# renjie-liang/HUAL

Measured on AMD Instinct MI355X. Metric: train clips/sec, higher is better.
Workload: dtype f32 (fp16x3 / bf16x3 split-operand MFMA, fp32 accumulate); 1 GPU; Charades-STA SeqPAN train step (fwd+bwd+clip+AdamWD, dropout 0.2), batch 64/GPU, T=128, vdim=1024, L=20, C=8, dim=128, 8 heads, 2 attention layers, random init; ONE batch resident in HBM, batch assembly (hual_assemble_batch) outside the timed region; global_batch=64, T=128, vdim=1024, L=20, parallelism=dp1, launch=hipGraph, video_dtype=f32

## Files before the change

### hual_amd/csrc/dablock.h

```cpp
#pragma once
#include "common.h"
#include "rowops.h"

namespace hual {

#define HUAL_LNPROJ_MAX 5
struct LnProjArgs {
  const float* x;
  const float* xa; int pre_site; float* x_out;
  uint8_t* pre_bits; uint8_t* y1_bits;
  const float* x2;
  const float* g1; const float* b1; float* y1;
  int drop_site1;
  const float* g2; const float* b2; float* y2;
  float* mean; float* rstd;
  int nproj;
  const float* wimg[HUAL_LNPROJ_MAX];
  const float* bias[HUAL_LNPROJ_MAX];
  float* out[HUAL_LNPROJ_MAX]; int ldo[HUAL_LNPROJ_MAX];
  int src[HUAL_LNPROJ_MAX];
  int accum[HUAL_LNPROJ_MAX];
  int act[HUAL_LNPROJ_MAX];
  int out_site[HUAL_LNPROJ_MAX];
  uint8_t* out_bits[HUAL_LNPROJ_MAX];
// ... 35 lines not shown
  int nsteps;
  const float* A[HUAL_LNBWD_MAX]; int lda[HUAL_LNBWD_MAX];
  const uint8_t* a_bits[HUAL_LNBWD_MAX];
  float* a_save[HUAL_LNBWD_MAX];
  const float* wimg_t[HUAL_LNBWD_MAX];
  int dst[HUAL_LNBWD_MAX];
  const float* add_dy1;
  const uint8_t* dy1_bits;
  const float* x; const float* mean; const float* rstd;
  const float* g1; const float* g2;
  const float* add1;
  float* dx;
  float* dz; const uint8_t* dz_bits;
  float* part;
  int R; int MT; uint32_t drop_row0;
  int Nv;
  const float* pre_x; const float* pre_mean; const float* pre_rstd; const float* pre_g; const float* pre_dy; const float* pre_add;
};
int ln_proj_bwd_rows(int R, int Nv = 0);
int ln_proj_bwd_blocks(int R, int Nv = 0);
int launch_ln_proj_bwd(const LnProjBwdArgs& a, const DropCfg& drop, hipStream_t s);

struct DaMidBwdArgs {
  const float* dz1;
  const float *gate, *val, *sg, *xg, *sv, *xv;
  const float* w[10];
  float *d_sc, *d_val, *d_ln1a, *d_g, *dz_sg, *dz_xg, *d_sv, *d_xv, *d_satt, *d_xatt;
  int R; int MT; int Nv;
};
int launch_da_mid_bwd(const DaMidBwdArgs& a, hipStream_t s);
bool ln2_mid_bwd_fits(const LnProjBwdArgs& a, const DaMidBwdArgs& m);
int launch_ln2_mid_bwd(const LnProjBwdArgs& a, const DaMidBwdArgs& m, const DropCfg& drop, hipStream_t s);

}
```

### hual_amd/csrc/dablock.hip

```cpp
#include "dablock.h"
#include "tilecore.h"
#include "prof.h"

using namespace hual;

__device__ __forceinline__ float4 sig4(float4 v) { return make_float4(sigmoidf_(v.x), sigmoidf_(v.y), sigmoidf_(v.z), sigmoidf_(v.w)); }

#include "lnproj_body.h"

template <int NT, bool PLAIN>
__global__ __launch_bounds__(CB_THREADS) void ln_proj_kernel(LnProjArgs a, DropCfg drop) {
  extern __shared__ __attribute__((aligned(16))) char lp_lds[];
  ln_proj_body<NT, false, PLAIN>(a, drop, lp_lds);
}
template <int NT>
__global__ __launch_bounds__(CB_THREADS) void ln_proj_pair_kernel(LnProjArgs a0, LnProjArgs a1, DropCfg drop) {
  extern __shared__ __attribute__((aligned(16))) char lp_lds[];
  if (blockIdx.y == 0) ln_proj_body<NT>(a0, drop, lp_lds);
  else ln_proj_body<NT>(a1, drop, lp_lds);
}

#define DA_ST_NT st4
#define DP_ROWS 48
#define DP_PLANE (DP_ROWS * 256)
// ... 248 lines not shown
    uint32_t nbe[NT];
#pragma unroll
    for (int rt = 0; rt < NT; ++rt) nbe[rt] = 15u;
    if (dr.enabled) drop_rows((uint32_t)(a.site + 4), a.bits4, nbe);
#pragma unroll
    for (int rt = 0; rt < NT; ++rt) {
      float4 v = addb(T1[rt], 8);
      if (dr.enabled) v = drop_scale(nbe[rt], v, dr.scale);
      v = cb_add(v, SV[rt]);
      save(a.out, rt, v);
      if (TAIL) scratch[(16 * rt + j) * 32 + (ecol >> 2)] = v;
    }
  }
  if (TAIL) {
    lds_barrier();
    ln_proj_body<NT, true, true>(*lp, drop, P1, r0, scratch, r0, 32, DP_ROWS, TP);
  }
}
template <int NT>
__global__ __launch_bounds__(CB_THREADS) void da_post_kernel(DaPostArgs a, DropCfg drop) {
  extern __shared__ __attribute__((aligned(16))) char dp_lds[];
  da_post_body<NT, false>(a, drop, nullptr, dp_lds);
}
template <int NT>
__global__ __launch_bounds__(CB_THREADS) void da_post_lnproj_kernel(DaPostArgs a, DropCfg drop, LnProjArgs lp) {
  extern __shared__ __attribute__((aligned(16))) char dp_lds[];
  da_post_body<NT, true>(a, drop, &lp, dp_lds);
}

#define LB_ROWS 48
#define LB_U (LB_ROWS / 16)
template <int NT> struct DaMidPre { TfW wa, wb; float4 gate[NT], val[NT]; };
#define LB_LDS ((size_t)4 * LB_ROWS * 256 + 8 * 4 * 32 * 16 + 2 * LB_ROWS * sizeof(float))
template <bool PRE, int NT, bool SIX, bool MID>
__device__ __forceinline__ bool ln_proj_bwd_body(const LnProjBwdArgs& a, const DropCfg& drop, char* lb_lds, const DaMidBwdArgs* m,
                                                 DaMidPre<NT>* mp, float4 (&zv)[LB_U]) {
  char* S0 = lb_lds;
  char* S1 = S0 + 2 * LB_ROWS * 256;
  char* Ps = S1 + 2 * LB_ROWS * 256;
  float* ainv0 = reinterpret_cast<float*>(Ps + 8 * 4 * 32 * 16);
  float* ainv1 = ainv0 + LB_ROWS;
  const int lane = threadIdx.x & 63, wave = threadIdx.x >> 6;
  const int l32 = threadIdx.x & 31, grp = threadIdx.x >> 5;
  const int col = 4 * l32;
  const int MT = a.MT, R = a.R;
  const int tile_ = xcd_tile_clip(blockIdx.x, R, a.Nv, MT);
  if (tile_ < 0) return false;
  const int r0 = tile_ * MT;
  const int RE = min(R, r0 + MT);
  const int j = lane & 15, g = lane >> 4, ecol = 16 * wave + 4 * g;
  const DropRegs dr = drop_load(drop);

  TfW w[2];
  tf_load_w(w[0], a.wimg_t[0], wave, lane);
  float4 nv[LB_U], xv[LB_U], a1v[LB_U];
  float mu[LB_U], rsd[LB_U];
  constexpr bool pre = PRE;
  const float* add1p = pre ? (a.pre_add ? a.pre_add : a.x) : (a.add1 ? a.add1 : a.x);
  const float* a0p = pre ? a.pre_dy : a.A[0];
  const int lda0 = pre ? HUAL_D : a.lda[0];
  uint32_t nkb[LB_U];
  const int nsteps = SIX ? 6 : (MID ? 1 : a.nsteps);
  auto has_bits = [&](int k) { return !SIX && a.a_bits[k] != nullptr; };
  auto to_second = [&](int k) { return SIX ? k >= 4 : a.dst[k] != 0; };
  const bool has_g2 = SIX || (!MID && a.g2 != nullptr), has_add_dy1 = SIX || (!MID && a.add_dy1 != nullptr), has_dy1_bits = !SIX && a.dy1_bits != nullptr;
  const uint8_t* kb0p = has_bits(0) ? a.a_bits[0] : reinterpret_cast<const uint8_t*>(a.x);
  float4 pxv[LB_U];
  float pmu[LB_U], prs[LB_U];
#pragma unroll
  for (int u = 0; u < LB_U; ++u) {
    const int row = min(r0 + grp + 16 * u, R - 1);
    nv[u] = ld4(a0p + (size_t)row * lda0 + col);
    nkb[u] = SIX ? 0u : kb0p[(size_t)row * 16 + (l32 >> 1)];
    xv[u] = ld4(a.x + (size_t)row * HUAL_D + col);
    a1v[u] = ld4(add1p + (size_t)row * HUAL_D + col);
    mu[u] = a.mean[row];
    rsd[u] = a.rstd[row];
    if (pre) { pxv[u] = ld4(a.pre_x + (size_t)row * HUAL_D + col); pmu[u] = a.pre_mean[row]; prs[u] = a.pre_rstd[row]; }
  }
  const float4 g1 = ld4(a.g1 + col);
  float4 sg2 = f4zero(), sb2 = f4zero();
  if (pre) {
    const float4 pg = ld4(a.pre_g + col);
#pragma unroll
    for (int u = 0; u < LB_U; ++u) {
      const int lr = grp + 16 * u;
      const bool ok = lr < MT && r0 + lr < RE;
      const float4 v = pxv[u], dy = nv[u];
      const float mean = pmu[u], rstd = prs[u];
      const float4 xh = make_float4((v.x - mean) * rstd, (v.y - mean) * rstd, (v.z - mean) * rstd, (v.w - mean) * rstd);
      if (ok) { sb2 = cb_add(sb2, dy); sg2 = cb_fma(dy, xh, sg2); }
      const float4 gv = cb_mul(dy, pg);
      const float m1 = fast_sum32(cb_hsum(gv)) * (1.0f / HUAL_D);
      const float m2 = fast_sum32(cb_hsum(cb_mul(gv, xh))) * (1.0f / HUAL_D);
      float4 dx = make_float4(rstd * (gv.x - m1 - xh.x * m2), rstd * (gv.y - m1 - xh.y * m2),
                              rstd * (gv.z - m1 - xh.z * m2), rstd * (gv.w - m1 - xh.w * m2));
      if (a.pre_add) dx = make_float4(__fadd_rn(dx.x, a1v[u].x), __fadd_rn(dx.y, a1v[u].y), __fadd_rn(dx.z, a1v[u].z), __fadd_rn(dx.w, a1v[u].w));
      nv[u] = dx;
      a1v[u] = dx;
    }
  }
  const float4 g2 = has_g2 ? ld4(a.g2 + col) : f4zero();
  float4 addt[NT];
  const float* addp = has_add_dy1 ? a.add_dy1 : a.x;
#pragma unroll
  for (int rt = 0; rt < NT; ++rt) addt[rt] = (SIX || MID) ? f4zero() : ld4(addp + (uint32_t)min(r0 + 16 * rt + j, R - 1) * (uint32_t)HUAL_D + (uint32_t)ecol);
  auto fill = [&](int k) {
    char* S = (k & 1) ? S1 : S0;
    float* ai = (k & 1) ? ainv1 : ainv0;
#pragma unroll
    for (int u = 0; u < LB_U; ++u) {
      const int lr = grp + 16 * u, row = r0 + lr;
      if (lr >= MT) continue;
      const bool ok = row < RE;
      float4 v = ok ? nv[u] : f4zero();
      if (has_bits(k)) {
// ... 326 lines not shown
  tf_mma_lean<NT, DP_PLANE>(P2, wb, lane, accp);
  tf_load_w(wb, a.w[9], wave, lane);
  fold(T2, ainv2, true);
#pragma unroll
  for (int rt = 0; rt < NT; ++rt) {
    T1[rt] = cb_add(T1[rt], U3[rt]);
    T2[rt] = cb_add(T2[rt], U4[rt]);
    save_nt(a.d_sv, rt, T1[rt]);
    save_nt(a.d_xv, rt, T2[rt]);
  }
  zero_invalid(T1);
  zero_invalid(T2);
  put_max(smaxA, T1);
  put_max(smaxB, T2);
  lds_barrier();
  put_planes(P1, ainv1, smaxA, T1);
  put_planes(P0, ainv0, smaxB, T2);
  lds_barrier();
  tf_mma_lean<NT, DP_PLANE>(P1, wa, lane, accp);
  fold(T1, ainv1, true);
#pragma unroll
  for (int rt = 0; rt < NT; ++rt) save(a.d_satt, rt, T1[rt]);
  tf_mma_lean<NT, DP_PLANE>(P0, wb, lane, accp);
  fold(T2, ainv0, true);
#pragma unroll
  for (int rt = 0; rt < NT; ++rt) save(a.d_xatt, rt, T2[rt]);
}
template <int NT>
__global__ __launch_bounds__(CB_THREADS) void da_mid_bwd_kernel(DaMidBwdArgs a) {
  extern __shared__ __attribute__((aligned(16))) char dm_lds[];
  const float4 zin[3] = {};
  da_mid_bwd_body<NT, false>(a, dm_lds, nullptr, zin);
}
template <int NT>
__global__ __launch_bounds__(CB_THREADS) void ln2_mid_bwd_kernel(LnProjBwdArgs a, DaMidBwdArgs m, DropCfg drop) {
  extern __shared__ __attribute__((aligned(16))) char lm_lds[];
  DaMidPre<NT> mp;
  float4 zv[LB_U];
  if (!ln_proj_bwd_body<false, NT, false, true>(a, drop, lm_lds, &m, &mp, zv)) return;
  static_assert(DP_SLOT == 2 * LB_ROWS * 256, "the middle's slot 1 must be the first body's slot 1");
  da_mid_bwd_body<NT, true>(m, lm_lds, &mp, zv);
}

#if defined(HUAL_STAMPS) && (HUAL_STAMPS == 1 || (HUAL_STAMPS >= 4 && HUAL_STAMPS <= 6))
extern "C" int hual_debug_stamps(unsigned long long* out, int n) {
  return (int)hipMemcpyFromSymbol(out, HIP_SYMBOL(g_hual_stamps), sizeof(unsigned long long) * (size_t)n);
}
extern "C" int hual_debug_stamps_reset() {
  static unsigned long long zeros[512 * HUAL_STAMP_SLOTS];
  return (int)hipMemcpyToSymbol(HIP_SYMBOL(g_hual_stamps), zeros, sizeof(zeros));
}
#endif

namespace hual {

static int tile_rows(int R, int Nv, int max_rows) { return xcd_clip_rows(R, Nv, 16, max_rows); }
int ln_proj_rows(int R, int Nv) { return tile_rows(R, Nv, LP_ROWS); }
int ln_proj_pair_rows(int R) {
  int mt = 16;
  while (mt < LP_ROWS && 2 * xcd_clip_grid(R, 0, mt) > 256) ++mt;
  return mt;
}
int da_post_rows(int R, int Nv) { return tile_rows(R, Nv, DP_ROWS); }

static int check_ln_proj(const LnProjArgs& a) {
  HUAL_REQUIRE(a.x && a.g1 && a.b1 && a.y1 && a.mean && a.rstd && a.R > 0, "ln_proj: null / empty");
// ... 156 lines not shown
  HUAL_CHECK_HIP(hipGetLastError());
  return 0;
}

static int check_da_mid_bwd(const DaMidBwdArgs& a) {
  HUAL_REQUIRE(a.dz1 && a.gate && a.val && a.sg && a.xg && a.sv && a.xv && a.R > 0, "da_mid_bwd: null / empty");
  HUAL_REQUIRE(a.MT >= 1 && a.MT <= DP_ROWS, "da_mid_bwd: MT must be 1..48");
  for (int k = 0; k < 10; ++k) HUAL_REQUIRE(a.w[k] != nullptr, "da_mid_bwd: null weight image");
  HUAL_REQUIRE(a.d_sc && a.d_val && a.d_ln1a && a.d_g && a.dz_sg && a.dz_xg && a.d_sv && a.d_xv && a.d_satt && a.d_xatt, "da_mid_bwd: null output");
  return 0;
}
static void da_mid_bwd_work(const DaMidBwdArgs& a, double& flops, double& bytes) {
  const double rows = (double)a.R;
  flops += 10.0 * 2.0 * rows * HUAL_D * HUAL_D;
  bytes += 4.0 * (rows * HUAL_D * 17.0 + 10.0 * HUAL_D * HUAL_D);
}

int launch_da_mid_bwd(const DaMidBwdArgs& a, hipStream_t s) {
  int rc = check_da_mid_bwd(a);
  if (rc) return rc;
  const size_t lds = DM_LDS;
  double flops = 0.0, bytes = 0.0;
  da_mid_bwd_work(a, flops, bytes);
  const dim3 grid(xcd_clip_grid(a.R, a.Nv, a.MT));
  switch (cdiv(a.MT, 16)) {
    case 1: { HUAL_DYN_LDS(da_mid_bwd_kernel<1>, 160 * 1024); HUAL_LAUNCH(flops, bytes, da_mid_bwd_kernel<1>, grid, dim3(CB_THREADS), lds, s, a); break; }
    case 2: { HUAL_DYN_LDS(da_mid_bwd_kernel<2>, 160 * 1024); HUAL_LAUNCH(flops, bytes, da_mid_bwd_kernel<2>, grid, dim3(CB_THREADS), lds, s, a); break; }
    default: { HUAL_DYN_LDS(da_mid_bwd_kernel<3>, 160 * 1024); HUAL_LAUNCH(flops, bytes, da_mid_bwd_kernel<3>, grid, dim3(CB_THREADS), lds, s, a); break; }
  }
  HUAL_CHECK_HIP(hipGetLastError());
  return 0;
}

bool ln2_mid_bwd_fits(const LnProjBwdArgs& a, const DaMidBwdArgs& m) {
  return a.nsteps == 1 && !a.pre_x && !a.g2 && !a.add_dy1 && a.dst[0] == 0 && a.dz && a.dz == m.dz1 && a.R == m.R && a.Nv == m.Nv && a.MT == m.MT;
}

int launch_ln2_mid_bwd(const LnProjBwdArgs& a, const DaMidBwdArgs& m, const DropCfg& drop, hipStream_t s) {
  int rc = check_ln_proj_bwd(a);
  if (rc) return rc;
  if ((rc = check_da_mid_bwd(m))) return rc;
  HUAL_REQUIRE(ln2_mid_bwd_fits(a, m), "ln2_mid_bwd: one product into one layer norm whose dz is the middle's dz1, on the same row tiles");
  static_assert(LB_ROWS == DP_ROWS, "the two bodies share their row tiles");
  const size_t lds = LB_LDS > DM_LDS ? LB_LDS : DM_LDS;
  double flops = 0.0, bytes = 0.0;
  ln_proj_bwd_work(a, flops, bytes);
  da_mid_bwd_work(m, flops, bytes);
  bytes -= 4.0 * (double)a.R * HUAL_D;
  const dim3 grid(xcd_clip_grid(a.R, a.Nv, a.MT));
  switch (cdiv(a.MT, 16)) {
    case 1: { HUAL_DYN_LDS(ln2_mid_bwd_kernel<1>, 160 * 1024); HUAL_LAUNCH(flops, bytes, ln2_mid_bwd_kernel<1>, grid, dim3(CB_THREADS), lds, s, a, m, drop); break; }
    case 2: { HUAL_DYN_LDS(ln2_mid_bwd_kernel<2>, 160 * 1024); HUAL_LAUNCH(flops, bytes, ln2_mid_bwd_kernel<2>, grid, dim3(CB_THREADS), lds, s, a, m, drop); break; }
    default: { HUAL_DYN_LDS(ln2_mid_bwd_kernel<3>, 160 * 1024); HUAL_LAUNCH(flops, bytes, ln2_mid_bwd_kernel<3>, grid, dim3(CB_THREADS), lds, s, a, m, drop); break; }
  }
  HUAL_CHECK_HIP(hipGetLastError());
  return 0;
}

}
```

### hual_amd/csrc/prof.cpp

```cpp
#include <stdlib.h>
#include "prof.h"
#include <map>
#include <string>
#include <vector>
#include <string.h>
#include "../../include/hual_seqpan.h"

namespace hual {

namespace {
struct Rec { std::string name; hipEvent_t a, b; double flops, bytes; };
struct Agg { std::string name; int64_t launches = 0; double usec = 0.0, flops = 0.0, bytes = 0.0; };
struct State {
  bool on = false;
  std::vector<Rec> recs;
  std::vector<Agg> aggs;
};
thread_local State g_prof;

std::string clean(const char* s) {
  std::string n(s);
  while (!n.empty() && (n.front() == '(' || n.front() == ' ')) n.erase(n.begin());
  while (!n.empty() && (n.back() == ')' || n.back() == ' ')) n.pop_back();
  return n;
// ... 39 lines not shown
    auto it = idx.find(r.name);
    if (it == idx.end()) {
      it = idx.emplace(r.name, g_prof.aggs.size()).first;
      g_prof.aggs.push_back(Agg{r.name});
    }
    Agg& a = g_prof.aggs[it->second];
    if (ok) { a.launches += 1; a.usec += (double)ms * 1e3; a.flops += r.flops; a.bytes += r.bytes; }
    hipEventDestroy(r.a);
    hipEventDestroy(r.b);
  }
  g_prof.recs.clear();
  return (int)g_prof.aggs.size();
}

int hual_prof_get(int i, char* name, int name_cap, int64_t* launches, double* usec, double* flops, double* bytes) {
  using namespace hual;
  if (i < 0 || i >= (int)g_prof.aggs.size() || !name || name_cap < 1) return HUAL_ERR_INVALID;
  const Agg& a = g_prof.aggs[i];
  strncpy(name, a.name.c_str(), (size_t)name_cap - 1);
  name[name_cap - 1] = 0;
  if (launches) *launches = a.launches;
  if (usec) *usec = a.usec;
  if (flops) *flops = a.flops;
  if (bytes) *bytes = a.bytes;
  return 0;
}

int hual_prof_kernel_pipe(const char* kernel, int* pipe, int* passes) {
  if (!kernel || !pipe || !passes) return HUAL_ERR_INVALID;
  struct Row { const char* prefix; int pipe, passes; };
  static const Row rows[] = {
      {"conv_block_", HUAL_PIPE_MATRIX16, 3}, {"ln_proj", HUAL_PIPE_MATRIX16, 3}, {"da_post", HUAL_PIPE_MATRIX16, 3},
      {"da_mid_bwd", HUAL_PIPE_MATRIX16, 3},  {"ln2_mid_bwd", HUAL_PIPE_MATRIX16, 3}, {"mproj_", HUAL_PIPE_MATRIX16, 3},
      {"feature_", HUAL_PIPE_MATRIX16, 3},    {"dw_f16_", HUAL_PIPE_MATRIX16, 3},
      {"attn_", HUAL_PIPE_MATRIX16, 3},      {"cq_fwd_staged", HUAL_PIPE_MATRIX16, 3}, {"cq_bwd_staged", HUAL_PIPE_MATRIX16, 3},
      {"cq_fwd_wide", HUAL_PIPE_MATRIX16, 3}, {"cq_bwd_wide", HUAL_PIPE_MATRIX16, 3},
      {"cq_", HUAL_PIPE_MATRIX32, 1},
  };
  for (const Row& r : rows)
    if (strncmp(kernel, r.prefix, strlen(r.prefix)) == 0) { *pipe = r.pipe; *passes = r.passes; return 0; }
  *pipe = HUAL_PIPE_NONE; *passes = 0;
  return 0;
}

}
```

### hual_amd/csrc/seqpan.hip

```cpp
#include "attn.h"
#include "prof.h"
#include "cq.h"
#include "convblock.h"
#include "dablock.h"
#include "embed.h"
#include "gemm.h"
#include "heads.h"
#include "mproj.h"
#include "optim.h"
#include "params.h"
#include "rowops.h"
#include <stdlib.h>
#include <string.h>
#include <algorithm>
#include <unordered_map>
#include <vector>

namespace hual {
const char* last_error_cstr();
}
using namespace hual;

namespace {

enum { ST_ALWAYS = 0, ST_INPUT = 1, ST_CONV = 2, ST_DA = 3, ST_CQ = 4, ST_FUSE = 5, ST_PRED = 6 };

struct WsEntry { std::string name; size_t off, rows, cols; };

struct Ctx {
  const hual_cfg* cfg = nullptr;
  ParamMap pm;
  int B = 0, T = 0, L = 0, C = 0;
  RowSpace rs;
  RowSpace rsv;
  char* base = nullptr;
  size_t cap = 0, used = 0;
  bool dry = true;
  hipStream_t stream = nullptr;
  DropCfg drop;
  const float* P = nullptr;
  float* G = nullptr;
  const float* word_table = nullptr;
  std::vector<WsEntry> entries;
  std::unordered_map<std::string, size_t> index;
  std::vector<DwJob> dwjobs;
  std::vector<ColsumJob> colsum;
  int rc = 0;
  bool static_tables = false;
  void* ext_table = nullptr; size_t ext_table_bytes = 0;
  int wall_K = 0; uint32_t wall_off = 0, wall_boff = 0;
  struct DenseW { size_t off; int K; size_t boff; uint8_t need; };
  bool ksplit = false;
  std::vector<DenseW> dense;
  char* PKF = nullptr;
  char* PKT = nullptr;
  char* PKN = nullptr;
  const float* timg(size_t off, int blk = 0) const { return reinterpret_cast<const float*>(PKT + boff_of(off) + (size_t)blk * 65536); }
  const float* nimg(size_t off, int blk = 0) const { return reinterpret_cast<const float*>(PKN + boff_of(off) + (size_t)blk * 65536); }
  size_t boff_of(size_t off) const {
    for (const auto& d : dense) if (d.off == off) return d.boff;
// ... 2 lines not shown
  size_t pk_bytes = 0;

  float* find(const std::string& name) {
    auto it = index.find(name);
    if (it != index.end()) return reinterpret_cast<float*>(base + entries[it->second].off);
    if (rc == 0) rc = fail(HUAL_ERR_WORKSPACE, "internal: unknown workspace buffer '" + name + "'");
    return reinterpret_cast<float*>(base);
  }
  float* buf(const std::string& name, size_t rows, size_t cols) {
    if (!dry || index.count(name)) return find(name);
    WsEntry e{name, used, rows, cols};
    size_t bytes = (rows * cols * sizeof(float) + 255) & ~(size_t)255;
    used += bytes + 256;
    index[name] = entries.size();
    entries.push_back(e);
    return reinterpret_cast<float*>(base + e.off);
  }
  float* act(const std::string& name) { return buf(name, (size_t)rs.R, HUAL_D); }
  int novf = 0;
  bool debug_taps = false;
  float* actv(const std::string& name) { return buf(name, (size_t)rs.Nv, HUAL_D); }
  float* vec(const std::string& name) { return buf(name, (size_t)rs.R, 1); }
  const float* p(size_t off) const { return P + off; }
  float* g(size_t off) const { return G + off; }
  int catw() const { return cfg->word_dim + 100; }
  bool ok() const { return rc == 0; }
  void chk(int r) { if (rc == 0 && r != 0) rc = r; }
  int sel_stage = -1, sel_sub = 0;
  bool active = true;
  bool want_bwd = false;
  int part_seq = 0;
  void stage(int st, int sub = 0) { active = sel_stage < 0 || st == ST_ALWAYS || (st == sel_stage && (st != ST_DA || sub == sel_sub)); }
  bool stage_on(int st, int sub = 0) const { return sel_stage < 0 || (st == sel_stage && (st != ST_DA || sub == sel_sub)); }
  bool live() const { return !dry && active && rc == 0; }
  void push_dw(const DwJob& j) { if (active) dwjobs.push_back(j); }

  void ln_bwd(const LnBwd& a0) {
    LnBwd a = a0;
    const int nblk = ln_bwd_blocks(a.R);
    a.part = buf("part." + std::to_string(part_seq++), (size_t)nblk * 4, HUAL_D);
    ColsumJob cj{};
    cj.src = a.part; cj.nblk = nblk; cj.nvec = 4;
    cj.dst[0] = a.dg1; cj.dst[1] = a.db1; cj.dst[2] = a.dg2; cj.dst[3] = a.db2;
    if (active) colsum.push_back(cj);
    if (live()) chk(launch_ln_bwd(a, drop, stream));
  }
  void ln_bwd_split(const LnBwd& a0, float* dg_lo, float* db_lo, float* dg_hi, float* db_hi, const PosBwdJob* pos = nullptr, int npos = 0) {
    LnBwd a = a0;
    const int nlo = ln_bwd_blocks(a.split), nhi = ln_bwd_blocks(a.R - a.split);
    a.part = buf("part." + std::to_string(part_seq++), (size_t)(nlo + nhi) * 4, HUAL_D);
    ColsumJob cj{};
    cj.src = a.part; cj.nblk = nlo; cj.nvec = 4;
    cj.dst[0] = dg_lo; cj.dst[1] = db_lo;
    if (active) colsum.push_back(cj);
    cj.src = a.part + (size_t)nlo * 4 * HUAL_D; cj.nblk = nhi;
    cj.dst[0] = dg_hi; cj.dst[1] = db_hi;
    if (active) colsum.push_back(cj);
    if (live()) chk(launch_ln_bwd(a, drop, stream, pos, npos, &rs));
  }
  void ln_proj_bwd(const LnProjBwdArgs& a0, float* dg1, float* db1, float* dg2, float* db2) {
    LnProjBwdArgs a = a0;
    a.MT = ln_proj_bwd_rows(a.R, a.Nv);
    const int nblk = ln_proj_bwd_blocks(a.R, a.Nv);
    a.part = buf("part." + std::to_string(part_seq++), (size_t)nblk * 4, HUAL_D);
    ColsumJob cj{};
    cj.src = a.part; cj.nblk = nblk; cj.nvec = 4;
    cj.dst[0] = dg1; cj.dst[1] = db1; cj.dst[2] = dg2; cj.dst[3] = db2;
    if (active) colsum.push_back(cj);
    if (live()) chk(launch_ln_proj_bwd(a, drop, stream));
  }
  void ln2_mid_bwd(const LnProjBwdArgs& a0, const DaMidBwdArgs& m0, float* dg1, float* db1) {
    LnProjBwdArgs a = a0;
    DaMidBwdArgs m = m0;
    a.MT = ln_proj_bwd_rows(a.R, a.Nv);
    m.MT = da_post_rows(m.R, m.Nv);
    const int nblk = ln_proj_bwd_blocks(a.R, a.Nv);
    a.part = buf("part." + std::to_string(part_seq++), (size_t)nblk * 4, HUAL_D);
    ColsumJob cj{};
    cj.src = a.part; cj.nblk = nblk; cj.nvec = 4;
    cj.dst[0] = dg1; cj.dst[1] = db1;
    if (active) colsum.push_back(cj);
    if (!live()) return;
#ifndef HUAL_NO_DA_BWD_FUSE
    if (sel_stage < 0 && ln2_mid_bwd_fits(a, m)) { chk(launch_ln2_mid_bwd(a, m, drop, stream)); return; }
#endif
    chk(launch_ln_proj_bwd(a, drop, stream));
    if (ok()) chk(launch_da_mid_bwd(m, stream));
  }
  void flush_colsum(const EmbedUnpack* unpack = nullptr) {
    for (size_t i = 0; i < colsum.size() && !dry && ok(); i += HUAL_COLSUM_MAX_JOBS) {
      const bool last = i + HUAL_COLSUM_MAX_JOBS >= colsum.size();
      chk(launch_colsum(colsum.data() + i, (int)std::min<size_t>(HUAL_COLSUM_MAX_JOBS, colsum.size() - i), stream, last ? unpack : nullptr));
    }
    if (colsum.empty() && unpack && !dry && ok()) chk(launch_colsum(nullptr, 0, stream, unpack));
    colsum.clear();
  }
  void attn_fwd(const AttnJob* j, int n) { if (live()) chk(launch_attn_fwd(j, n, drop, stream)); }
  void attn_bwd(const AttnJob* j, int n) {
    if (live()) chk(launch_attn_bwd(j, n, drop, stream));
  }
};

void set_embed_scratch(EmbedArgs& ea, float* base, int Nq, int C, int char_dim) {
  const EmbedLayout el = embed_layout(Nq, C, char_dim);
  ea.cemb = base + el.cemb; ea.ball = base + el.ball;
  ea.yall = base + el.yall; ea.dxall = base + el.dxall; ea.dfall = base + el.dfall;
}
void fill_embed_args(Ctx& c, EmbedArgs& ea, const hual_batch* bt, float* cat, int catw, int32_t* char_arg, float* scratch) {
  const ParamMap& pm = c.pm;
  ea.word_ids = bt->word_ids; ea.char_ids = bt->char_ids; ea.word_table = c.word_table; ea.unk = c.p(pm.unk);
  ea.char_table = c.p(pm.char_table);
  for (int i = 0; i < 4; ++i) { ea.filt[i] = c.p(pm.filt[i]); ea.fbias[i] = c.p(pm.fbias[i]); }
  ea.cat = cat; ea.ldcat = catw; ea.char_arg = char_arg;
  set_embed_scratch(ea, scratch, c.rs.Nq, c.C, c.cfg->char_dim);
  ea.word_dim = c.cfg->word_dim; ea.char_dim = c.cfg->char_dim; ea.C = c.C; ea.num_chars = c.cfg->num_chars;
  ea.wall_img = reinterpret_cast<const float*>(c.PKT + c.wall_boff);
  ea.wall_img_t = reinterpret_cast<const float*>(c.PKN + c.wall_boff);
}
DwJob mkdw(const float* A, int lda, int K, const float* dY, int ldy, int M, float* dW, float* db, int N = HUAL_D) {
  DwJob j;
  dw_job_init(j);
  j.npieces = 1;
  j.A[0] = A; j.lda[0] = lda; j.kw[0] = K; j.dW[0] = dW; j.ldw = N;
  j.dY = dY; j.ldy = ldy; j.M = M; j.N = N; j.db = db;
  return j;
}

MProjStep mstep(const float* A, int lda, int kw, const float* img, int wrows, bool first, bool last) {
  MProjStep s{};
  s.A = A; s.lda = lda; s.kw = kw; s.wimg = img; s.wrows = wrows; s.first = first ? 1 : 0; s.last = last ? 1 : 0;
  s.drop_site = -1; s.rep = 1; s.add_div = 1; s.ncol = HUAL_D;
  return s;
}
MProjStep mstep_reuse(const float* img, int wrows, bool first, bool last) {
  MProjStep s = mstep(nullptr, 0, 0, img, wrows, first, last);
  s.reuse = 1;
  return s;
}
void mstep_out(MProjStep& s, float* out, int ldo, const float* bias = nullptr, int ncol = HUAL_D) { s.out = out; s.ldo = ldo; s.bias = bias; s.ncol = ncol; }
MProjArgs margs(int R, int R_other = 0) {
  MProjArgs a{};
  a.R = R; a.MT = mproj_rows(R, R_other); a.drop_row0 = 0;
  return a;
}

void flush_dw(Ctx& c) {
  const size_t n = c.dwjobs.size();
  if (n == 0) return;
  std::stable_sort(c.dwjobs.begin(), c.dwjobs.end(), [](const DwJob& a, const DwJob& b) { return a.M > b.M; });
  DwJob* table = reinterpret_cast<DwJob*>(c.buf("dw.table.0", 1, dw_table_words(n)));
  if (!c.dry && c.ext_table) {
    if (4 * dw_table_words(n) > c.ext_table_bytes) { c.chk(fail(HUAL_ERR_INVALID, "hual_run_opts.dw_table too small: hual_seqpan_dw_table_bytes()")); return; }
    table = reinterpret_cast<DwJob*>(c.ext_table);
  }
  if (!c.dry && c.ok()) c.chk(launch_dw(c.dwjobs.data(), (int)n, c.drop, c.stream, table, !c.static_tables));
  c.dwjobs.clear();
}

int setup_ctx(Ctx& c, const hual_cfg* cfg, int B, int T, int L, int C) {
  HUAL_REQUIRE(cfg != nullptr, "null cfg");
  int rc = build_param_map(*cfg, c.pm);
  if (rc) return rc;
  HUAL_REQUIRE(B >= 1 && T >= 1 && L >= 1, "empty batch");
  HUAL_REQUIRE(T <= cfg->max_vlen && L <= cfg->max_vlen, "sequence longer than max_vlen (assert_less_equal, modules.py:44)");
  HUAL_REQUIRE(T <= 256 && L <= 256, "T, L <= 256");
  HUAL_REQUIRE(C >= 4, "char_ids need C >= 4 (conv width 4, VALID)");
  HUAL_REQUIRE((long long)B * (T + L) * 8 < (1ll << 28), "batch too large for 32-bit RNG row ids");
  HUAL_REQUIRE((long long)B * (T + L) < (1ll << 20), "batch too large: B (T + L) < 2^20 rows (row -> clip lookups, common.h small_div)");
  c.cfg = cfg; c.B = B; c.T = T; c.L = L; c.C = C;
  {
    const ParamMap& pm = c.pm;
    const int D = HUAL_D, catw = cfg->word_dim + 100;
    c.dense.clear();
    const uint8_t TN = HUAL_PACK_T | HUAL_PACK_N;
    auto add = [&](size_t off, int K, uint8_t need) { if (K % 8 == 0) c.dense.push_back({off, K, off * 4, need}); };
    const int qks = ((catw + 3) / 4 + 63) & ~63;
    c.ksplit = (cfg->vdim % 256) == 0 && cfg->vdim <= 1024 && (catw % 8) == 0 && qks <= 256;
    add(pm.vconv.k, cfg->vdim, c.ksplit ? HUAL_PACK_F : HUAL_PACK_T);
    add(pm.qconv.k, catw, (c.ksplit ? HUAL_PACK_F : HUAL_PACK_T) | HUAL_PACK_N);
    add(pm.shid.k, 2 * D, TN); add(pm.ehid.k, 2 * D, TN);
// ... 539 lines not shown
  return c.rc;
}


struct HeadGrads { float *d_fn[2], *d_out; };
HeadGrads bwd_heads(Ctx& c, const HeadBufs& b, float* outputs) {
  const ParamMap& pm = c.pm;
  const int D = HUAL_D, Nv = c.rs.Nv, B = c.B;
  if (c.live() && c.sel_stage >= 0) {
    HeadsArgs ha{};
    ha.grad_only = 1; ha.h[0] = b.h[0]; ha.h[1] = b.h[1]; ha.w[0] = c.p(pm.sdense.k); ha.w[1] = c.p(pm.edense.k); ha.b[0] = c.p(pm.sdense.b); ha.b[1] = c.p(pm.edense.b);
    ha.ds = b.d_logit[0]; ha.de = b.d_logit[1]; ha.dZ[0] = b.dz[0]; ha.dZ[1] = b.dz[1]; ha.part[0] = b.part[0]; ha.part[1] = b.part[1];
    c.chk(launch_heads(ha, B, c.T, c.stream));
  }
  for (int h = 0; h < 2; ++h) {
    ColsumJob cj{};
    cj.src = b.part[h]; cj.nblk = B; cj.nvec = 2; cj.last_ncols = 1;
    cj.dst[0] = c.g(h == 0 ? pm.sdense.k : pm.edense.k); cj.dst[1] = c.g(h == 0 ? pm.sdense.b : pm.edense.b);
    if (c.active) c.colsum.push_back(cj);
    const DenseP& hp = h == 0 ? pm.shid : pm.ehid;
    DwJob j = mkdw(b.fn[h], D, D, b.dz[h], D, Nv, c.g(hp.k), c.g(hp.b));
    j.npieces = 2; j.A[1] = outputs; j.lda[1] = D; j.kw[1] = D; j.dW[1] = c.g(hp.k) + (size_t)D * D;
    c.push_dw(j);
  }
  HeadGrads g{};
  g.d_fn[0] = c.actv("d.head.sfn"); g.d_fn[1] = c.actv("d.head.efn"); g.d_out = c.actv("d.outputs.heads");
  if (c.live()) {
    MProjArgs pr = margs(Nv);
    pr.nsteps = 4;
    pr.s[0] = mstep(b.dz[0], D, D, c.nimg(pm.shid.k, 0), D, true, true);     mstep_out(pr.s[0], g.d_fn[0], D);
    pr.s[1] = mstep_reuse(c.nimg(pm.shid.k, 1), D, true, false);
    pr.s[2] = mstep(b.dz[1], D, D, c.nimg(pm.ehid.k, 1), D, false, true);    mstep_out(pr.s[2], g.d_out, D);
    pr.s[3] = mstep_reuse(c.nimg(pm.ehid.k, 0), D, true, true);             mstep_out(pr.s[3], g.d_fn[1], D);
    c.chk(launch_mproj(&pr, 1, c.drop, c.stream));
  }
  return g;
}

float* bwd_fe(Ctx& c, int ps, const HeadBufs& hd, float* d_fn, float* d_in) {
  const ParamMap& pm = c.pm;
  const int D = HUAL_D, Nv = c.rs.Nv;
  const std::string dt = "d.fe" + std::to_string(ps);
  const FeBufs b = fe_bufs(Res{c, false}, ps);
  float* f = b.cb.x[4];
  float* dzd = c.actv(dt + ".zd");
  c.push_dw(mkdw(b.l2, D, D, dzd, D, Nv, c.g(pm.fe_dense.k), c.g(pm.fe_dense.b)));
  float* d_res = c.actv(dt + ".res");
  float* d_att = c.actv(dt + ".att");
  {
    LnProjBwdArgs lb{};
    const LnP& hl = ps == 1 ? pm.eln : pm.sln;
    lb.pre_x = b.out; lb.pre_mean = hd.mean + (ps == 1 ? Nv : 0); lb.pre_rstd = hd.rstd + (ps == 1 ? Nv : 0);
    lb.pre_g = c.p(hl.g); lb.pre_dy = d_fn; lb.pre_add = ps == 1 ? nullptr : d_in;
    lb.a_bits[0] = b.kb8; lb.a_save[0] = dzd;
    lb.nsteps = 1; lb.A[0] = nullptr; lb.lda[0] = D; lb.wimg_t[0] = c.nimg(pm.fe_dense.k); lb.dst[0] = 0;
    lb.dy1_bits = b.kb7; lb.x = b.res; lb.mean = b.mean2; lb.rstd = b.rstd2; lb.g1 = c.p(pm.fe_ln2.g);
    lb.dx = d_res; lb.dz = d_att; lb.dz_bits = b.kb6; lb.R = Nv; lb.drop_row0 = 0;
    c.ln_proj_bwd(lb, c.g(pm.fe_ln2.g), c.g(pm.fe_ln2.b), c.g(hl.g), c.g(hl.b));
  }
  float* d_qkv = c.buf(dt + ".qkv", Nv, 3 * D);
  AttnJob a = b.job;
  a.dO = d_att; a.lddo = D; a.dQ = d_qkv; a.lddq = 3 * D; a.dK = d_qkv + D; a.dV = d_qkv + 2 * D; a.lddkv = 3 * D;
  c.attn_bwd(&a, 1);
  const DenseP* pr[3] = {&pm.fe_q, &pm.fe_k, &pm.fe_v};
  for (int k = 0; k < 3; ++k) c.push_dw(mkdw(b.a, D, D, d_qkv + k * D, 3 * D, Nv, c.g(pr[k]->k), c.g(pr[k]->b)));
  float* d_f = c.actv(dt + ".x4");
  {
// ... 242 lines not shown
    eu.a = ea; eu.g = eg; eu.CP = embed_unpack_cpad(ea); eu.ntasks = embed_unpack_tasks(ea);
    eu.finish_blocks = embed_finish_blocks(ea, c.rs.Nq); eu.finish_lds = embed_finish_lds(ea); eu.nrows = c.rs.Nq; eu.drop = c.drop;
  }
  c.flush_colsum(unpack ? &eu : nullptr);
}

int backward_graph(Ctx& c, const hual_batch* bt, const hual_labels* lab, const hual_run_opts* opt) {
  const Res r{c, false};
  c.dwjobs.clear(); c.colsum.clear(); c.part_seq = 0;
  c.stage(ST_ALWAYS);
  const CoreBufs core = core_bufs(r);
  const InputBufs in = input_bufs(r);
  const CqStage cq = cq_bufs(r, r.act("da" + std::to_string(c.cfg->attn_layer - 1) + ".out"));
  const FuseBufs fu = fuse_bufs(r, cq.feats, lab);
  const HeadBufs hd = head_bufs(r);
  {
    const bool prezeroed = !c.dry && opt->prezero_token && *opt->prezero_token == (uint64_t)(uintptr_t)c.G && c.sel_stage < 0;
    if (!c.dry && opt->prezero_token) *opt->prezero_token = 0;
    if (c.live() && !prezeroed) c.chk(launch_zero(c.G, c.pm.total, c.stream));
  }
  c.stage(ST_PRED);
  const HeadGrads hg = bwd_heads(c, hd, fu.outputs);
  float* fe_dx0[2] = {nullptr, nullptr};
  fe_dx0[1] = bwd_fe(c, 1, hd, hg.d_fn[1], nullptr);
  fe_dx0[0] = bwd_fe(c, 0, hd, hg.d_fn[0], fe_dx0[1]);
  float* d_cqf = bwd_fuse(c, core, fu, hd, cq.feats, fe_dx0[0], hg.d_out, lab, opt);
  float* dx = bwd_cq(c, cq, d_cqf);
  for (int li = c.cfg->attn_layer - 1; li >= 0; --li) dx = bwd_da(c, li, dx);
  c.stage(ST_CONV);
  float* d_x0 = conv_block_bwd(c, cb_bufs(r, "cb", in.x0, c.rs.R), dx, c.pm.cb, c.rs);
  EmbedArgs ea{}; EmbedGrads eg{};
  const bool input_ran = bwd_input(c, in, d_x0, fe_dx0, bt, ea, eg);
  bwd_flush(c, ea, eg, input_ran);
  return c.rc;
}

int plan(Ctx& c, const hual_cfg* cfg, int B, int T, int L, int C) {
  int rc = setup_ctx(c, cfg, B, T, L, C);
  if (rc) return rc;
  c.dry = true;
  c.base = nullptr;
  hual_run_opts o{};
  rc = forward_graph(c, nullptr, nullptr, nullptr, &o);
  if (rc) return rc;
  return backward_graph(c, nullptr, nullptr, &o);
}

}

extern "C" {

int hual_seqpan_validate(const hual_cfg* cfg) {
  HUAL_REQUIRE(cfg != nullptr, "null cfg");
  return validate_cfg(*cfg);
}

#define HUAL_DW_TABLE_JOBS 256
uint64_t hual_seqpan_dw_table_bytes(void) { return 4 * dw_table_words(HUAL_DW_TABLE_JOBS); }

int hual_seqpan_param_count(const hual_cfg* cfg, uint64_t* padded_floats, uint64_t* count) {
  HUAL_REQUIRE(cfg != nullptr, "null cfg");
  ParamMap pm;
  int rc = build_param_map(*cfg, pm);
  if (rc) return rc;
  if (padded_floats) *padded_floats = pm.total;
  if (count) *count = pm.count;
// ... 277 lines not shown
```

Before: 54150 clips/s.

## Fuse prediction-head dx products into the first feature-encoder LN-projection backward kernel

The four head-gradient matrix products (d_fn0, d_out, d_fn1), previously run in a separate mproj launch, are deferred and computed as a prologue inside the ln_proj_bwd kernel of the end-side feature encoder. The d_fn1 result stays in LDS and feeds the PRE layernorm backward directly, so one launch is removed along with the global write and reread of d_fn1. In exchange the kernel needs extra LDS and more work per block, and it adds deferred-launch bookkeeping to the Ctx with flush points wherever ordering matters.

```diff
diff --git a/hual_amd/csrc/dablock.h b/hual_amd/csrc/dablock.h
--- a/hual_amd/csrc/dablock.h
+++ b/hual_amd/csrc/dablock.h
@@ -91,4 +91,13 @@
 bool ln2_mid_bwd_fits(const LnProjBwdArgs& a, const DaMidBwdArgs& m);
 int launch_ln2_mid_bwd(const LnProjBwdArgs& a, const DaMidBwdArgs& m, const DropCfg& drop, hipStream_t s);
 
+struct HeadsDxArgs {
+  const float* dz[2];
+  const float* w[4];
+  float *d_fn0, *d_out, *d_fn1;
+  int R; int MT;
+};
+bool heads_fe_bwd_fits(const HeadsDxArgs& h, const LnProjBwdArgs& a);
+int launch_heads_fe_bwd(const HeadsDxArgs& h, const LnProjBwdArgs& a, const DropCfg& drop, hipStream_t s);
+
 }
diff --git a/hual_amd/csrc/dablock.hip b/hual_amd/csrc/dablock.hip
--- a/hual_amd/csrc/dablock.hip
+++ b/hual_amd/csrc/dablock.hip
@@ -304,9 +304,12 @@
 #define LB_U (LB_ROWS / 16)
 template <int NT> struct DaMidPre { TfW wa, wb; float4 gate[NT], val[NT]; };
 #define LB_LDS ((size_t)4 * LB_ROWS * 256 + 8 * 4 * 32 * 16 + 2 * LB_ROWS * sizeof(float))
-template <bool PRE, int NT, bool SIX, bool MID>
+#define LB_DY_OFF LB_LDS
+#define LB_LDS_HEADS (LB_LDS + (size_t)LB_ROWS * 512)
+template <bool PRE, int NT, bool SIX, bool MID, bool HEADS = false>
 __device__ __forceinline__ bool ln_proj_bwd_body(const LnProjBwdArgs& a, const DropCfg& drop, char* lb_lds, const DaMidBwdArgs* m,
-                                                 DaMidPre<NT>* mp, float4 (&zv)[LB_U]) {
+                                                 DaMidPre<NT>* mp, float4 (&zv)[LB_U], const HeadsDxArgs* hx = nullptr) {
+  static_assert(!HEADS || (PRE && !SIX && !MID), "the heads' products go in front of the PRE form");
   char* S0 = lb_lds;
   char* S1 = S0 + 2 * LB_ROWS * 256;
   char* Ps = S1 + 2 * LB_ROWS * 256;
@@ -324,7 +327,19 @@
   const DropRegs dr = drop_load(drop);
 
   TfW w[2];
-  tf_load_w(w[0], a.wimg_t[0], wave, lane);
+  float4 hz0[LB_U], hz1[LB_U];
+  if (HEADS) {
+    tf_load_w(w[0], hx->w[0], wave, lane);
+#pragma unroll
+    for (int u = 0; u < LB_U; ++u) {
+      const size_t off = (size_t)min(r0 + grp + 16 * u, R - 1) * HUAL_D + col;
+      hz0[u] = ld4(hx->dz[0] + off);
+      hz1[u] = ld4(hx->dz[1] + off);
+    }
+    tf_load_w(w[1], hx->w[1], wave, lane);
+  } else {
+    tf_load_w(w[0], a.wimg_t[0], wave, lane);
+  }
   float4 nv[LB_U], xv[LB_U], a1v[LB_U];
   float mu[LB_U], rsd[LB_U];
   constexpr bool pre = PRE;
@@ -342,7 +357,7 @@
 #pragma unroll
   for (int u = 0; u < LB_U; ++u) {
     const int row = min(r0 + grp + 16 * u, R - 1);
-    nv[u] = ld4(a0p + (size_t)row * lda0 + col);
+    if (!HEADS) nv[u] = ld4(a0p + (size_t)row * lda0 + col);
     nkb[u] = SIX ? 0u : kb0p[(size_t)row * 16 + (l32 >> 1)];
     xv[u] = ld4(a.x + (size_t)row * HUAL_D + col);
     a1v[u] = ld4(add1p + (size_t)row * HUAL_D + col);
@@ -352,8 +367,48 @@
   }
   const float4 g1 = ld4(a.g1 + col);
   float4 sg2 = f4zero(), sb2 = f4zero();
+  float4 pgh = f4zero();
+  if (HEADS) {
+    pgh = ld4(a.pre_g + col);
+#pragma unroll
+    for (int u = 0; u < LB_U; ++u) {
+      const int lr = grp + 16 * u;
+      if (lr >= MT) continue;
+      const bool ok = r0 + lr < RE;
+      const float i0 = cb_store_operand(S0, S0 + LB_ROWS * 256, lr, l32, ok ? hz0[u] : f4zero());
+      const float i1 = cb_store_operand(S1, S1 + LB_ROWS * 256, lr, l32, ok ? hz1[u] : f4zero());
+      if (l32 == 0) { ainv0[lr] = ok ? i0 : 0.f; ainv1[lr] = ok ? i1 : 0.f; }
+    }
+    lds_barrier();
+    float4* DY = reinterpret_cast<float4*>(lb_lds + LB_DY_OFF);
+    f32x4 hp[NT];
+    float4 ho[NT];
+    auto scaled = [&](const f32x4& p, float ir, float4 o) { return make_float4(fmaf(p[0], ir, o.x), fmaf(p[1], ir, o.y), fmaf(p[2], ir, o.z), fmaf(p[3], ir, o.w)); };
+    auto save = [&](float* dst, int rt, float4 v) {
+      const int row = r0 + 16 * rt + j;
+      if (row < RE) st4(dst + (uint32_t)row * (uint32_t)HUAL_D + (uint32_t)ecol, v);
+    };
+    tf_mma_lean<NT, LB_ROWS * 256>(S0, w[0], lane, hp);
+    tf_load_w(w[0], hx->w[2], wave, lane);
+#pragma unroll
+    for (int rt = 0; rt < NT; ++rt) save(hx->d_fn0, rt, scaled(hp[rt], ainv0[16 * rt + j], f4zero()));
+    tf_mma_lean<NT, LB_ROWS * 256>(S0, w[1], lane, hp);
+    tf_load_w(w[1], hx->w[3], wave, lane);
+#pragma unroll
+    for (int rt = 0; rt < NT; ++rt) ho[rt] = scaled(hp[rt], ainv0[16 * rt + j], f4zero());
+    tf_mma_lean<NT, LB_ROWS * 256>(S1, w[0], lane, hp);
+    tf_load_w(w[0], a.wimg_t[0], wave, lane);
+#pragma unroll
+    for (int rt = 0; rt < NT; ++rt) save(hx->d_out, rt, scaled(hp[rt], ainv1[16 * rt + j], ho[rt]));
+    tf_mma_lean<NT, LB_ROWS * 256>(S1, w[1], lane, hp);
+#pragma unroll
+    for (int rt = 0; rt < NT; ++rt) DY[(16 * rt + j) * 32 + (ecol >> 2)] = scaled(hp[rt], ainv1[16 * rt + j], f4zero());
+    lds_barrier();
+#pragma unroll
+    for (int u = 0; u < LB_U; ++u) nv[u] = DY[(grp + 16 * u) * 32 + l32];
+  }
   if (pre) {
-    const float4 pg = ld4(a.pre_g + col);
+    const float4 pg = HEADS ? pgh : ld4(a.pre_g + col);
 #pragma unroll
     for (int u = 0; u < LB_U; ++u) {
       const int lr = grp + 16 * u;
@@ -746,6 +801,13 @@
   const float4 zin[3] = {};
   da_mid_bwd_body<NT, false>(a, dm_lds, nullptr, zin);
 }
+template <int NT>
+__global__ __launch_bounds__(CB_THREADS) void heads_fe_bwd_kernel(HeadsDxArgs h, LnProjBwdArgs a, DropCfg drop) {
+  extern __shared__ __attribute__((aligned(16))) char hf_lds[];
+  float4 zv[LB_U];
+  ln_proj_bwd_body<true, NT, false, false, true>(a, drop, hf_lds, nullptr, nullptr, zv, &h);
+}
+
 template <int NT>
 __global__ __launch_bounds__(CB_THREADS) void ln2_mid_bwd_kernel(LnProjBwdArgs a, DaMidBwdArgs m, DropCfg drop) {
   extern __shared__ __attribute__((aligned(16))) char lm_lds[];
@@ -968,6 +1030,33 @@
   return 0;
 }
 
+bool heads_fe_bwd_fits(const HeadsDxArgs& h, const LnProjBwdArgs& a) {
+  return a.nsteps == 1 && a.pre_x && a.pre_dy && a.pre_dy == h.d_fn1 && !a.pre_add && !a.g2 && !a.add1 && !a.add_dy1 && a.dst[0] == 0 &&
+         a.R == h.R && a.Nv == 0 && a.MT == h.MT && a.MT <= LB_ROWS;
+}
+
+int launch_heads_fe_bwd(const HeadsDxArgs& h, const LnProjBwdArgs& a, const DropCfg& drop, hipStream_t s) {
+  int rc = check_ln_proj_bwd(a);
+  if (rc) return rc;
+  HUAL_REQUIRE(h.dz[0] && h.dz[1] && h.w[0] && h.w[1] && h.w[2] && h.w[3] && h.d_fn0 && h.d_out, "heads_fe_bwd: null tensor");
+  HUAL_REQUIRE(heads_fe_bwd_fits(h, a), "heads_fe_bwd: the one-product PRE form whose pre_dy is the heads' d_fn1, on the same row tiles");
+  const size_t lds = LB_LDS_HEADS;
+  double flops = 0.0, bytes = 0.0;
+  ln_proj_bwd_work(a, flops, bytes);
+  const double rows = (double)a.R;
+  flops += 4.0 * 2.0 * rows * HUAL_D * HUAL_D;
+  bytes += 4.0 * (rows * HUAL_D * 4.0 + 4.0 * HUAL_D * HUAL_D);
+  bytes -= 4.0 * rows * HUAL_D;
+  const dim3 grid(xcd_clip_grid(a.R, a.Nv, a.MT));
+  switch (cdiv(a.MT, 16)) {
+    case 1: { HUAL_DYN_LDS(heads_fe_bwd_kernel<1>, 160 * 1024); HUAL_LAUNCH(flops, bytes, heads_fe_bwd_kernel<1>, grid, dim3(CB_THREADS), lds, s, h, a, drop); break; }
+    case 2: { HUAL_DYN_LDS(heads_fe_bwd_kernel<2>, 160 * 1024); HUAL_LAUNCH(flops, bytes, heads_fe_bwd_kernel<2>, grid, dim3(CB_THREADS), lds, s, h, a, drop); break; }
+    default: { HUAL_DYN_LDS(heads_fe_bwd_kernel<3>, 160 * 1024); HUAL_LAUNCH(flops, bytes, heads_fe_bwd_kernel<3>, grid, dim3(CB_THREADS), lds, s, h, a, drop); break; }
+  }
+  HUAL_CHECK_HIP(hipGetLastError());
+  return 0;
+}
+
 bool ln2_mid_bwd_fits(const LnProjBwdArgs& a, const DaMidBwdArgs& m) {
   return a.nsteps == 1 && !a.pre_x && !a.g2 && !a.add_dy1 && a.dst[0] == 0 && a.dz && a.dz == m.dz1 && a.R == m.R && a.Nv == m.Nv && a.MT == m.MT;
 }
diff --git a/hual_amd/csrc/prof.cpp b/hual_amd/csrc/prof.cpp
--- a/hual_amd/csrc/prof.cpp
+++ b/hual_amd/csrc/prof.cpp
@@ -95,6 +95,7 @@
   static const Row rows[] = {
       {"conv_block_", HUAL_PIPE_MATRIX16, 3}, {"ln_proj", HUAL_PIPE_MATRIX16, 3}, {"da_post", HUAL_PIPE_MATRIX16, 3},
       {"da_mid_bwd", HUAL_PIPE_MATRIX16, 3},  {"ln2_mid_bwd", HUAL_PIPE_MATRIX16, 3}, {"mproj_", HUAL_PIPE_MATRIX16, 3},
+      {"heads_fe_bwd", HUAL_PIPE_MATRIX16, 3},
       {"feature_", HUAL_PIPE_MATRIX16, 3},    {"dw_f16_", HUAL_PIPE_MATRIX16, 3},
       {"attn_", HUAL_PIPE_MATRIX16, 3},      {"cq_fwd_staged", HUAL_PIPE_MATRIX16, 3}, {"cq_bwd_staged", HUAL_PIPE_MATRIX16, 3},
       {"cq_fwd_wide", HUAL_PIPE_MATRIX16, 3}, {"cq_bwd_wide", HUAL_PIPE_MATRIX16, 3},
diff --git a/hual_amd/csrc/seqpan.hip b/hual_amd/csrc/seqpan.hip
--- a/hual_amd/csrc/seqpan.hip
+++ b/hual_amd/csrc/seqpan.hip
@@ -26,6 +26,8 @@
 enum { ST_ALWAYS = 0, ST_INPUT = 1, ST_CONV = 2, ST_DA = 3, ST_CQ = 4, ST_FUSE = 5, ST_PRED = 6 };
 
 struct WsEntry { std::string name; size_t off, rows, cols; };
+
+bool cb_no_tail();
 
 struct Ctx {
   const hual_cfg* cfg = nullptr;
@@ -94,9 +96,21 @@
   int part_seq = 0;
   void stage(int st, int sub = 0) { active = sel_stage < 0 || st == ST_ALWAYS || (st == sel_stage && (st != ST_DA || sub == sel_sub)); }
   bool stage_on(int st, int sub = 0) const { return sel_stage < 0 || (st == sel_stage && (st != ST_DA || sub == sel_sub)); }
-  bool live() const { return !dry && active && rc == 0; }
+  bool on() const { return !dry && active && rc == 0; }
+  bool live() { if (!on()) return false; flush_pending(); return on(); }
   void push_dw(const DwJob& j) { if (active) dwjobs.push_back(j); }
 
+  bool pend_heads = false;
+  MProjArgs pend_mp; HeadsDxArgs pend_hx;
+  void defer_heads_dx(const MProjArgs& mp, const HeadsDxArgs& hx) {
+    if (!live()) return;
+    pend_mp = mp; pend_hx = hx; pend_heads = true;
+  }
+  void flush_pending() {
+    if (!pend_heads) return;
+    pend_heads = false;
+    if (rc == 0) chk(launch_mproj(&pend_mp, 1, drop, stream));
+  }
   void ln_bwd(const LnBwd& a0) {
     LnBwd a = a0;
     const int nblk = ln_bwd_blocks(a.R);
@@ -129,6 +143,14 @@
     cj.src = a.part; cj.nblk = nblk; cj.nvec = 4;
     cj.dst[0] = dg1; cj.dst[1] = db1; cj.dst[2] = dg2; cj.dst[3] = db2;
     if (active) colsum.push_back(cj);
+    if (!on()) return;
+#ifndef HUAL_NO_HEADS_FE_BWD_FUSE
+    if (pend_heads && sel_stage < 0 && !cb_no_tail() && heads_fe_bwd_fits(pend_hx, a)) {
+      pend_heads = false;
+      chk(launch_heads_fe_bwd(pend_hx, a, drop, stream));
+      return;
+    }
+#endif
     if (live()) chk(launch_ln_proj_bwd(a, drop, stream));
   }
   void ln2_mid_bwd(const LnProjBwdArgs& a0, const DaMidBwdArgs& m0, float* dg1, float* db1) {
@@ -150,6 +172,7 @@
     if (ok()) chk(launch_da_mid_bwd(m, stream));
   }
   void flush_colsum(const EmbedUnpack* unpack = nullptr) {
+    flush_pending();
     for (size_t i = 0; i < colsum.size() && !dry && ok(); i += HUAL_COLSUM_MAX_JOBS) {
       const bool last = i + HUAL_COLSUM_MAX_JOBS >= colsum.size();
       chk(launch_colsum(colsum.data() + i, (int)std::min<size_t>(HUAL_COLSUM_MAX_JOBS, colsum.size() - i), stream, last ? unpack : nullptr));
@@ -208,6 +231,7 @@
 
 void flush_dw(Ctx& c) {
   const size_t n = c.dwjobs.size();
+  c.flush_pending();
   if (n == 0) return;
   std::stable_sort(c.dwjobs.begin(), c.dwjobs.end(), [](const DwJob& a, const DwJob& b) { return a.M > b.M; });
   DwJob* table = reinterpret_cast<DwJob*>(c.buf("dw.table.0", 1, dw_table_words(n)));
@@ -813,7 +837,12 @@
     pr.s[1] = mstep_reuse(c.nimg(pm.shid.k, 1), D, true, false);
     pr.s[2] = mstep(b.dz[1], D, D, c.nimg(pm.ehid.k, 1), D, false, true);    mstep_out(pr.s[2], g.d_out, D);
     pr.s[3] = mstep_reuse(c.nimg(pm.ehid.k, 0), D, true, true);             mstep_out(pr.s[3], g.d_fn[1], D);
-    c.chk(launch_mproj(&pr, 1, c.drop, c.stream));
+    HeadsDxArgs hx{};
+    hx.dz[0] = b.dz[0]; hx.dz[1] = b.dz[1];
+    hx.w[0] = pr.s[0].wimg; hx.w[1] = pr.s[1].wimg; hx.w[2] = pr.s[2].wimg; hx.w[3] = pr.s[3].wimg;
+    hx.d_fn0 = g.d_fn[0]; hx.d_out = g.d_out; hx.d_fn1 = g.d_fn[1]; hx.R = Nv; hx.MT = pr.MT;
+    if (c.sel_stage < 0) c.defer_heads_dx(pr, hx);
+    else c.chk(launch_mproj(&pr, 1, c.drop, c.stream));
   }
   return g;
 }
@@ -1122,6 +1151,7 @@
   EmbedArgs ea{}; EmbedGrads eg{};
   const bool input_ran = bwd_input(c, in, d_x0, fe_dx0, bt, ea, eg);
   bwd_flush(c, ea, eg, input_ran);
+  c.flush_pending();
   return c.rc;
 }
 
```

Result: no change. 54290 clips/s (median of 6 runs) (+0.3%).
